# rsokolovskii/fl_scaling_sc_ldpc

Measured on AMD Instinct MI355X. Metric: MC codeword trials/sec, (4,8) SC-LDPC L=50 N=1000 eps=0.48 full BP, higher is better.
Workload: dtype u32

## Files before the change

### fl_scaling_sc_ldpc_amd/csrc/full_bp_small.hip

```cpp
#include "common.h"
#include "kernel_util.h"
#include "table_rows.h"
#include <algorithm>
#include <cstdlib>
#include <type_traits>

namespace {

using namespace scldpc_dev;

enum { SC_NE = 0, SC_REM, SC_N0, SC_N1, SC_OVF, SC_Q, SC_N = 8 };
enum { LV_VALID = 2, LV_EXTRA0 = 3, LV_PUSH = 6, LV_DROP = 9, LV_REM = 12, LV_OVF = 15, LV_N = 18 };

struct SmArgs {
    int L, V, C, n, nk, cn_lim, nw, ncw;
    uint32_t magic_v, magic_c;
    int ntrials;
    int kswitch;
    int max_it;
    int rows_cap;
    int32_t *rows;
    int off_U, off_q0, off_q1, off_pos, off_scal, off_fb, total, qcap;
    const uint16_t *vn_adj16;
    const uint16_t *cn_adj16;
    const uint32_t *chan;
    int32_t *counters;
    uint32_t *erased_out;
    int ncaps;
    int caps[SCLDPC_MAX_CAPS];
};


template <int BLOCK, bool LEVEL, bool PERSIST, bool SOCK, bool TRAJ = false, bool CAPS = false, bool WIDE = false, int DV = 4, int DC = 8,
          int OCC = 0>
__global__ __launch_bounds__(BLOCK, OCC ? OCC : WIDE ? 4 : PERSIST ? 8 : 7) __attribute__((amdgpu_num_sgpr(96))) void full_bp_small_kernel(const SmArgs a)
{
    static_assert(!WIDE || (BLOCK == 1024 && LEVEL && SOCK && !PERSIST), "the wide form: LEVEL [+ TRAJ | CAPS], socket table");
    static_assert(!(TRAJ && CAPS), "the checkpoints have no rows form");
    static_assert((DV == 4 && DC == 8) || (SOCK && !PERSIST), "other degree pairs: the socket table, no PERSIST");
    static_assert(DC <= 15 && DC % 2 == 0 && DV < DC, "a CN's count of erased neighbours is a nibble; CN rows are read as 32-bit words");
    using QT = std::conditional_t<WIDE, uint32_t, uint16_t>;
    constexpr int kWaves = BLOCK / 64;
    extern __shared__ uint32_t lds[];
    uint32_t *cnt = lds;
    uint32_t *U = lds + a.off_U;
    QT *q[2] = {reinterpret_cast<QT *>(lds + a.off_q0), reinterpret_cast<QT *>(lds + a.off_q1)};
    int *pos_cnt = reinterpret_cast<int *>(lds + a.off_pos);
    int *pos_ss = pos_cnt + a.L;
    int *scal = reinterpret_cast<int *>(lds + a.off_scal);

    const int tid = threadIdx.x, lane = tid & 63, wave = tid >> 6;
    auto decode_trial = [&](const int trial) {
    STAMP_DECL
    const int n = a.n, nk = a.nk, cn_lim = a.cn_lim, nw = a.nw, V = a.V, C = a.C, L = a.L, qcap = a.qcap;
    const auto *vrow = reinterpret_cast<const typename VnUnit<DV>::type *>(a.vn_adj16) + (size_t)trial * n * VnUnit<DV>::per_row;
    const auto *crow = reinterpret_cast<const typename CnUnit<DC>::type *>(a.cn_adj16) + (size_t)trial * nk * CnUnit<DC>::per_row;
    auto vn_row = [&](int j) { if constexpr (DV == 4) return load_row(vrow, j); else return load_row<DV>(vrow, j); };
    auto cn_row = [&](int c) { if constexpr (DC == 8) return load_row(crow, c); else return load_row<DC>(crow, c); };
    const uint32_t *ch = a.chan + (size_t)trial * nw;

    for (int c = tid; c < a.ncw; c += BLOCK) cnt[c] = 0;
    int ne_local = 0;
    for (int w = tid; w < nw; w += BLOCK) {
        const uint32_t x = chan_tail(ch[w], w, nw, n);
        U[w] = x;
        ne_local += __popc(x);
    }
    if (tid < LV_N) scal[tid] = 0;
    for (int i = tid; i < 2 * L; i += BLOCK) pos_cnt[i] = 0;
    __syncthreads();
    ne_local = wave_sum(ne_local);
    if (lane == 0 && ne_local) atomicAdd(&scal[SC_NE], ne_local);

    constexpr int NB = 8;
    for (int j0 = tid; j0 < n; j0 += NB * BLOCK) {
        Row<DV> r[NB];
        bool er[NB];
#pragma unroll
        for (int u = 0; u < NB; u++) {
            const int j = j0 + u * BLOCK;
            er[u] = false;
            if (j < n) { r[u] = vn_row(j); er[u] = (U[j >> 5] >> (j & 31)) & 1u; }
        }
#pragma unroll
        for (int u = 0; u < NB; u++) {
            const int j = j0 + u * BLOCK;
            if (er[u]) {
                const int base = (int)__umulhi((uint32_t)j, a.magic_v) * C;
                int cc[DV];
#pragma unroll
                for (int i = 0; i < DV; i++) cc[i] = base + i * C + (int)r[u][i];
#pragma unroll
                for (int i = 0; i < DV; i++) atomicAdd(&cnt[cc[i] >> 3], 1u << ((cc[i] & 7) * 4));
            }
        }
    }
    __syncthreads();
    STAMP(0);
    const int nch = scal[SC_NE];

    int removed = 0, drops = 0;
    auto step = [&](int c, uint32_t (&out)[DV]) {
#pragma unroll
        for (int i = 0; i < DV; i++) out[i] = 0;
        const Row<DC> s = cn_row(c);
        uint32_t jk[DC];
        bool none[DC];
#pragma unroll
        for (int k = 0; k < DC; k++) { jk[k] = s[k]; none[k] = jk[k] == 0xFFFFu; }
        if constexpr (SOCK) {
            const int vbase = (int)__umulhi((uint32_t)c, a.magic_c) * V;
#pragma unroll
            for (int k = 0; k < DC; k++) jk[k] = (uint32_t)(vbase - (int)(jk[k] % DV) * V) + (jk[k] / DV);
        }
        uint32_t wd[DC];
#pragma unroll
        for (int k = 0; k < DC; k++) wd[k] = U[none[k] ? 0u : jk[k] >> 5];
        int j = -1;
#pragma unroll
        for (int k = 0; k < DC; k++)
            if (!none[k] && ((wd[k] >> (jk[k] & 31u)) & 1u)) j = (int)jk[k];
        if (j < 0) return;
        const Row<DV> r = vn_row(j);
        const uint32_t bit = 1u << (j & 31);
        if (!(atomicAnd(&U[j >> 5], ~bit) & bit)) return;
        removed++;
        const int base = (int)__umulhi((uint32_t)j, a.magic_v) * C;
        int cc[DV];
#pragma unroll
        for (int i = 0; i < DV; i++) cc[i] = base + i * C + (int)r[i];
        uint32_t o[DV];
#pragma unroll
        for (int i = 0; i < DV; i++) o[i] = atomicSub(&cnt[cc[i] >> 3], 1u << ((cc[i] & 7) * 4));
#pragma unroll
        for (int i = 0; i < DV; i++) {
            const uint32_t old = (o[i] >> ((cc[i] & 7) * 4)) & 15u;
            if (old == 2u && cc[i] < cn_lim) out[i] = (uint32_t)cc[i] + 1u;
            if constexpr (LEVEL) drops += (old == 1u && cc[i] < cn_lim);
        }
    };
    auto ones_of = [&](int w) {
        const uint32_t y = cnt[w] ^ 0x11111111u;
        uint32_t z = ~(((y & 0x77777777u) + 0x77777777u) | y) & 0x88888888u;
        if (w * 8 + 8 > cn_lim) {
            const int keep = cn_lim - w * 8;
            z = keep <= 0 ? 0u : (z & ((1u << (4 * keep)) - 1u));
        }
        return z;
    };
    auto append = [&](const uint32_t (&out)[DV], int *push, QT *qn, bool &overflow) {
        int mine = 0;
#pragma unroll
        for (int i = 0; i < DV; i++) mine += out[i] != 0u;
        const int incl = (int)wave_inclusive_scan((uint32_t)mine);
        const int tot = __builtin_amdgcn_readlane(incl, 63);
        if (tot) {
            int base = 0;
            if (lane == 0) base = atomicAdd(push, tot);
            int idx = __builtin_amdgcn_readfirstlane(base) + incl - mine;
#pragma unroll
            for (int i = 0; i < DV; i++)
                if (out[i]) { if (idx < qcap) qn[idx] = (QT)(out[i] - 1u); else overflow = true; idx++; }
        }
    };

    int rounds = 0, ne = 0, status = 0, be = 0, ee = 0, bee = 0;
    auto residual = [&]() {
    if (ne > 0) {
        for (int w = tid; w < nw; w += BLOCK) {
            uint32_t x = U[w];
            int p0 = (int)__umulhi((uint32_t)(w * 32), a.magic_v);
            int room = (p0 + 1) * V - w * 32;
            while (x) {
                const uint32_t lo = room >= 32 ? x : (x & ((1u << room) - 1u));
                if (lo) atomicAdd(&pos_cnt[p0], __popc(lo));
                x = room >= 32 ? 0u : (x >> room);
                p0++;
                room = V;
            }
        }
        __syncthreads();
        int q0 = 0;
        for (;;) {
            while (q0 < L && pos_cnt[q0] == 0) q0++;
            if (q0 >= L) break;
            for (int t = tid; t < V; t += BLOCK) {
                const int j = q0 * V + t;
                if (!((U[j >> 5] >> (j & 31)) & 1u)) continue;
                const Row<DV> r = vn_row(j);
                const int base = q0 * C;
                int cc[DV];
#pragma unroll
                for (int i = 0; i < DV; i++) cc[i] = base + i * C + (int)r[i];
                bool pair = true;
#pragma unroll
                for (int i = 0; i < DV; i++) pair = pair && ((cnt[cc[i] >> 3] >> ((cc[i] & 7) * 4)) & 15u) == 2u;
                if (!pair) continue;
                int partner = -1;
                for (int i = 0; i < DV && pair; i++) {
                    const Row<DC> s = cn_row(cc[i]);
                    int other = -1;
                    for (int k = 0; k < DC; k++) {
                        const uint32_t jk = s[k];
                        if (jk == 0xFFFFu) continue;
                        const int j2 = SOCK ? (q0 + i - (int)(jk % DV)) * V + (int)(jk / DV) : (int)jk;
                        if (j2 != j && ((U[j2 >> 5] >> (j2 & 31)) & 1u)) other = j2;
                    }
                    if (other < 0 || (i > 0 && other != partner)) pair = false;
                    partner = other;
                }
                if (pair && (int)__umulhi((uint32_t)partner, a.magic_v) == q0) atomicAdd(&pos_ss[q0], 1);
            }
            __syncthreads();
            const int e = pos_cnt[q0] - pos_ss[q0];
            if (e > 0) { ee = e; bee = 1; break; }
            q0++;
        }
        for (int pos = 0; pos < L; pos++) be += pos_cnt[pos] > 0;
    }
    };
    auto put = [&](int32_t *o, int ne, int be, int ee, int bee, int rounds, int status) {
        o[SCLDPC_C_NUM_ERASURES] = ne;
        o[SCLDPC_C_NUM_BLOCKS_ERR] = be;
        o[SCLDPC_C_NUM_ERASURES_EXP] = ee;
        o[SCLDPC_C_NUM_BLOCKS_ERR_EXP] = bee;
        o[SCLDPC_C_NUM_ERASURES_P1] = 0;
        o[SCLDPC_C_ITERATIONS] = rounds;
        o[SCLDPC_C_STATUS] = status;
        o[SCLDPC_C_CHANNEL_ERASURES] = nch;
    };
    auto cap_counters = [&](int k) { return a.counters + ((size_t)k * a.ntrials + trial) * SCLDPC_NCOUNTERS; };

    int ci = 0;
    if constexpr (LEVEL) {
        uint8_t *fb = reinterpret_cast<uint8_t *>(lds + a.off_fb);
        int prec = n, iter = 0, ncur = 0, nfront = 0, first_word = 0;
        if constexpr (TRAJ) {
            int extra = 0;
            const int head = (DV - 1) * C, tail0 = L * C;
            for (int i = tid; i < 2 * head; i += BLOCK) {
                const int c = i < head ? i : tail0 + (i - head);
                if (c >= cn_lim || c >= nk) continue;
                const Row<DC> s = cn_row(c);
                int deg = 0;
#pragma unroll
                for (int k = 0; k < DC; k++) deg += s[k] != 0xFFFFu;
                extra += deg == 1 && ((cnt[c >> 3] >> ((c & 7) * 4)) & 15u) == 0u;
            }
            extra = wave_sum(extra);
            if (lane == 0 && extra) atomicAdd(&scal[LV_EXTRA0], extra);
        }
        bool scan = true;
        ne = nch;
        for (;;) {
            const int g = iter % 3, gn = (iter + 1) % 3;
            QT *qc = q[iter & 1], *qn = q[(iter + 1) & 1];
            if (tid == 0) { scal[LV_PUSH + gn] = 0; scal[LV_DROP + gn] = 0; scal[LV_REM + gn] = 0; scal[LV_OVF + gn] = 0; }
            int *push = &scal[LV_PUSH + g];
            bool overflow = false;
            removed = 0; drops = 0;
            auto run_queue = [&](int nq) {
                for (int k0 = wave * 64; k0 < nq; k0 += BLOCK) {
                    uint32_t out[DV] = {};
                    if (k0 + lane < nq) step((int)qc[k0 + lane], out);
                    append(out, push, qn, overflow);
                }
            };
            if (scan) {
                int valid = 0;
                for (int w = tid; w < a.ncw; w += BLOCK) {
                    uint32_t y = ones_of(w) >> 3;
                    y = (y | (y >> 3)) & 0x03030303u;
                    y = (y | (y >> 6)) & 0x000F000Fu;
                    y = (y | (y >> 12)) & 0xFFu;
                    fb[w] = (uint8_t)y;
                    valid += __popc(y);
                }
                if (iter == 0) {
                    valid = wave_sum(valid);
                    if (lane == 0 && valid) atomicAdd(&scal[LV_VALID], valid);
                }
                if (tid == 0) scal[SC_Q] = 0;
                __syncthreads();
                if (iter == 0) nfront = scal[LV_VALID];
                for (;;) {
                    for (int w0 = wave * 64; w0 < a.ncw; w0 += BLOCK) {
                        const int w = w0 + lane;
                        uint32_t y = w < a.ncw ? (uint32_t)fb[w] : 0u;
                        const int mine = __popc(y);
                        const int incl = (int)wave_inclusive_scan((uint32_t)mine);
                        const int tot = __builtin_amdgcn_readlane(incl, 63);
                        if (tot == 0) continue;
                        int base = 0;
                        if (lane == 0) base = atomicAdd(&scal[SC_Q], tot);
                        int idx = __builtin_amdgcn_readfirstlane(base) + incl - mine;
                        uint32_t left = 0;
                        while (y) {
                            const int k = __ffs((int)y) - 1;
                            y &= y - 1;
                            if (idx < qcap) qc[idx] = (QT)(w * 8 + k); else left |= 1u << k;
                            idx++;
                        }
                        if (mine) fb[w] = (uint8_t)left;
                    }
                    __syncthreads();
                    const int found = scal[SC_Q];
                    __syncthreads();
                    if (tid == 0) scal[SC_Q] = 0;
                    run_queue(min(found, qcap));
                    if (found <= qcap) break;
                    __syncthreads();
                }
            } else {
                run_queue(ncur);
            }
            STAMP(4);
            {
                const uint32_t both = (uint32_t)wave_sum((int)((uint32_t)removed | ((uint32_t)drops << 15)));
                removed = (int)(both & 0x7FFFu); drops = (int)(both >> 15);
            }
            if (lane == 0) {
                if (removed) atomicAdd(&scal[LV_REM + g], removed);
                if (drops) atomicAdd(&scal[LV_DROP + g], drops);
            }
            if (overflow) scal[LV_OVF + g] = 1;
            STAMP(5);
            __syncthreads();
            STAMP(6);
            const int deg1 = nfront + ((TRAJ && iter == 0) ? scal[LV_EXTRA0] : 0);
            ne -= scal[LV_REM + g];
            const int recovered = prec - ne;
            if constexpr (TRAJ) {
                if (wave == 0 && a.rows && rounds < a.rows_cap) {
                    int fw = first_word, first = n;
                    while (fw < nw) {
                        const uint32_t w = (fw + lane < nw) ? U[fw + lane] : 0u;
                        const unsigned long long m = __ballot(w != 0u);
                        if (m) {
                            const int l0 = __ffsll((long long)m) - 1;
                            const uint32_t w0 = (uint32_t)__shfl((int)w, l0, 64);
                            fw += l0;
                            first = fw * 32 + (__ffs((int)w0) - 1);
                            break;
                        }
                        fw += 64;
                    }
                    first_word = fw;
                    if (lane == 0) {
                        int32_t *r = a.rows + ((size_t)trial * a.rows_cap + rounds) * 3;
                        r[0] = deg1; r[1] = recovered; r[2] = (int)__umulhi((uint32_t)first, a.magic_v);
                    }
                }
                __syncthreads();
            }
            rounds++;
            if (deg1 < recovered && iter > 0) { status = -1; break; }
            if (ne == 0 || ne == prec) break;
            prec = ne;
            nfront = scal[LV_PUSH + g] - (scal[LV_DROP + g] - nfront);
            scan = scal[LV_OVF + g] != 0;
            ncur = scan ? 0 : scal[LV_PUSH + g];
            iter++;
            if (!CAPS && a.max_it > 0 && iter >= a.max_it) break;
            if constexpr (CAPS) {
                if (iter >= a.caps[ci]) {
                    be = ee = bee = 0;
                    residual();
                    if (tid == 0) put(cap_counters(ci), ne, be, ee, bee, rounds, 0);
                    __syncthreads();
                    for (int i = tid; i < 2 * L; i += BLOCK) pos_cnt[i] = 0;
                    if (++ci == a.ncaps) break;
                }
            }
            STAMP(7);
        }
        __syncthreads();
        STAMP(1);
    } else {
        const int kSwitch = a.kswitch;
        const int wcap = (qcap / kWaves) & ~1, half_cap = wcap / 2;
        int ncur = 0;
        bool scan = true;
        for (;;) {
            QT *qc = q[rounds & 1], *qn = q[(rounds + 1) & 1];
            if (scan) {
                for (int w0 = wave * 64; w0 < a.ncw; w0 += BLOCK) {
                    const int w = w0 + lane;
                    uint32_t z = w < a.ncw ? ones_of(w) : 0u;
                    const int mine = __popc(z);
                    const int incl = (int)wave_inclusive_scan((uint32_t)mine);
                    const int tot = __builtin_amdgcn_readlane(incl, 63);
                    if (tot == 0) continue;
                    int base = 0;
                    if (lane == 0) base = atomicAdd(&scal[SC_Q], tot);
                    base = __builtin_amdgcn_readfirstlane(base);
                    int idx = base + incl - mine;
                    while (z) {
                        const int k = (__ffs((int)z) - 1) >> 2;
                        z &= z - 1;
                        if (idx < qcap) qc[idx] = (QT)(w * 8 + k);
                        idx++;
                    }
                }
                __syncthreads();
                ncur = scal[SC_Q];
                if (ncur > qcap) { ncur = qcap; if (tid == 0) scal[SC_OVF] = 1; }
                __syncthreads();
            }
            if (tid == 0) { scal[SC_Q] = 0; scal[SC_N0 + ((rounds + 1) & 1)] = 0; }
            int *push = &scal[SC_N0 + (rounds & 1)];
            bool overflow = false;
            if (ncur > kSwitch || half_cap < 64) {
                for (int k0 = wave * 64; k0 < ncur; k0 += BLOCK) {
                    uint32_t out[DV] = {};
                    if (k0 + lane < ncur) step((int)qc[k0 + lane], out);
                    append(out, push, qn, overflow);
                }
            } else {
                QT *mine = qn + wave * wcap;
                int cntw = (ncur - wave + kWaves - 1) / kWaves, cur = 0;
                if (cntw < 0) cntw = 0;
                if (lane < cntw) mine[lane] = qc[wave + lane * kWaves];
                while (cntw > 0) {
                    QT *src = mine + cur * half_cap, *dst = mine + (cur ^ 1) * half_cap;
                    int ncnt = 0;
                    for (int b0 = 0; b0 < cntw; b0 += 64) {
                        uint32_t out[DV] = {};
                        if (b0 + lane < cntw) step((int)src[b0 + lane], out);
                        {
                            int mine_n = 0;
    #pragma unroll
                            for (int i = 0; i < DV; i++) mine_n += out[i] != 0u;
                            const int incl = (int)wave_inclusive_scan((uint32_t)mine_n);
                            int idx = ncnt + incl - mine_n;
    #pragma unroll
                            for (int i = 0; i < DV; i++)
                                if (out[i]) { if (idx < half_cap) dst[idx] = (QT)(out[i] - 1u); else overflow = true; idx++; }
                            ncnt += __builtin_amdgcn_readlane(incl, 63);
                        }
                    }
                    cntw = min(ncnt, half_cap);
                    cur ^= 1;
                }
            }
            if (overflow) scal[SC_OVF] = 1;
            __syncthreads();
            rounds++;
            const int pushed = *push;
            scan = scal[SC_OVF] != 0;
            __syncthreads();
            if (tid == 0) scal[SC_OVF] = 0;
            ncur = scan ? 0 : min(pushed, qcap);
            if (!scan && ncur == 0) break;
        }
        STAMP(1);
        removed = wave_sum(removed);
        if (lane == 0 && removed) atomicAdd(&scal[SC_REM], removed);
        __syncthreads();
        ne = nch - scal[SC_REM];
    }

    if (!CAPS || ci < a.ncaps) {
        be = ee = bee = 0;
        residual();
    }
    STAMP(2);
    STAMP_FLUSH();
    if (a.erased_out)
        for (int w = tid; w < nw; w += BLOCK) a.erased_out[(size_t)trial * nw + w] = U[w];
    if (tid == 0) {
        if constexpr (CAPS) {
            for (int k = ci; k < a.ncaps; k++) put(cap_counters(k), ne, be, ee, bee, rounds, status);
        } else {
            put(a.counters + (size_t)trial * SCLDPC_NCOUNTERS, ne, be, ee, bee, rounds, status);
        }
    }
    };
    if constexpr (PERSIST) {
        for (int trial = blockIdx.x; trial < a.ntrials; trial += gridDim.x) {
            decode_trial(trial);
            __syncthreads();
        }
    } else {
        decode_trial((int)blockIdx.x);
    }
}

int make_args(const scldpc_code_params *p, int32_t is_term, SmArgs *a, int per_cu, bool level = false, bool wide = false)
{
    const int n = scldpc::n_of(p), nk = scldpc::nk_of(p);
    a->L = p->L; a->V = p->vns_pos; a->C = p->cns_pos; a->n = n; a->nk = nk;
    a->cn_lim = is_term ? nk : p->L * p->cns_pos;
    a->nw = (n + 31) / 32; a->ncw = (nk + 7) / 8;
    int off = 0;
    auto take = [&](int words) { int o = off; off += (words + 3) & ~3; return o; };
    take(a->ncw);
    a->off_U = take(a->nw);
    a->off_pos = take(2 * p->L);
    a->off_scal = take(LV_N);
    a->off_fb = level ? take((a->ncw + 3) / 4) : 0;
    const int budget = scldpc::kMaxLdsBytes / per_cu / 4 - 128;
    int qwords = ((budget - off) / 2) & ~3;
    if (qwords > 2048 && !wide) qwords = 2048;
    if (qwords < 128) return -1;
    a->qcap = wide ? qwords : 2 * qwords;
    a->off_q0 = take(qwords);
    a->off_q1 = take(qwords);
    a->total = off;
    return 0;
}

constexpr int kBlockSmall = 256;
constexpr int kPerCu = 7;
constexpr int kSwitchWidth = 128;
constexpr int kBlockWide = 1024;
constexpr int kWideMinQueue = 1024;
static_assert(kSwitchWidth <= 64 * (kBlockSmall / 64), "a wave takes at most one frontier entry per lane into its private queue");

constexpr int pair_of(int dv, int dc) { return dv == 4 && dc == 8 ? 0 : dv == 3 && dc == 6 ? 1 : dv == 5 && dc == 10 ? 2 : -1; }

int carve(const scldpc_code_params *p, int32_t is_term, bool level, bool wide, SmArgs *a, int per_cu = kPerCu)
{
    if (wide) per_cu = 1;
    while (per_cu > 1 && make_args(p, is_term, a, per_cu, level, wide) != 0) per_cu--;
    return make_args(p, is_term, a, per_cu, level, wide) == 0 ? per_cu : -1;
}

const char *shape_limit(const scldpc_code_params *p, bool wide, bool sock, bool deg = false)
{
    if (scldpc::check_params(p)) return "invalid code parameters";
    if (!deg) {
        if (p->dv != 4 || p->dc != 8) return "takes dv = 4, dc = 8 only";
    } else {
        if (p->dc > 15) return "dc must be at most 15 (a CN's count of erased neighbours is kept in 4 bits)";
        if (pair_of(p->dv, p->dc) < 0) {
            static thread_local char text[96];
            snprintf(text, sizeof text, "no instance for dv = %d, dc = %d (takes (3,6), (4,8) and (5,10))", p->dv, p->dc);
            return text;
        }
    }
    if (sock && (int64_t)p->vns_pos * p->dv > 65535) return "sockets: vns_pos * dv must fit 16 bits (at most 65535)";
    if (p->cns_pos > 65536) return "at most 65536 CNs per position (16-bit position-local CN ids)";
    const int64_t n64 = (int64_t)p->L * p->vns_pos, nk64 = (int64_t)(p->L + p->dv - 1) * p->cns_pos;
    if (!wide && nk64 > 65536) return "at most 65536 CNs per trial (16-bit queue entries; the _wide forms take more)";
    if (!sock && n64 >= 65535) return "global VN ids in the CN -> VN table: fewer than 65535 VNs (use the _sock16 form beyond)";
    if (n64 / 8 + nk64 / 2 > scldpc::kMaxLdsBytes) return "LDS: the CN counts and VN bits of a trial exceed 160 KiB";
    SmArgs a{};
    uint32_t m;
    if (!scldpc::magic_of(p->vns_pos, scldpc::n_of(p) + 32, &m) || !scldpc::magic_of(p->cns_pos, scldpc::nk_of(p), &m))
        return "no exact multiply-high division for this vns_pos / cns_pos";
    if (make_args(p, 1, &a, 1, wide, wide) != 0) return "LDS: the CN counts and VN bits of a trial leave no room for the queues";
    if (wide && a.qcap < kWideMinQueue) return "queue: the LDS left by the state holds fewer than 1024 entries per queue";
    if (wide && a.nk / 16 + 64 * (a.nk / a.qcap + 1) > 32767) return "queue: a wave's releases per iteration could exceed 15 bits";
    if (deg) {
        if (!wide && carve(p, 1, true, false, &a) < 0) return "LDS: the CN counts and VN bits of a trial leave no room for the queues";
        const int r = a.nk / (wide ? kBlockWide / 64 : kBlockSmall / 64) + 64 * (a.nk / a.qcap + 1);
        if (r > 32767) return "queue: a wave's releases per iteration could exceed 15 bits";
        if (p->dv * r >= (1 << 17)) return "queue: the CNs a wave zeroes per iteration could exceed 17 bits";
    }
    return nullptr;
}

}

const char *scldpc::small_deg_shape_limit(const scldpc_code_params *p) { return shape_limit(p, false, true, true); }

extern "C" int scldpc_full_bp_wide_supported(const scldpc_code_params *p) { return shape_limit(p, true, true) == nullptr; }

extern "C" int scldpc_full_bp_cn16_supported(const scldpc_code_params *p) { return shape_limit(p, false, false) == nullptr; }

extern "C" int scldpc_full_bp_sock16_supported(const scldpc_code_params *p) { return shape_limit(p, false, true) == nullptr; }

namespace {

enum Mode { M_FIX, M_LEVEL, M_TRAJ, M_CAPS };
constexpr bool kCnTable = false, kSockTable = true, kNarrow = false, kWide = true, kDeg = true;
struct Form {
    Mode mode;
    bool sock;
    bool wide;
    bool deg = false;
    bool knobs() const { return mode != M_CAPS && !wide && !deg; }
};

struct Call {
    const scldpc_code_params *p;
    int32_t ntrials;
    const uint16_t *vn_adj16, *cn_adj16;
    const uint32_t *chan;
    int32_t max_it, is_term;
    int32_t *counters;
    uint32_t *erased;
    void *stream;
    int32_t *rows; int32_t rows_cap;
    int32_t ncaps; const int32_t *caps;
};

using Kernel = void (*)(const SmArgs);
constexpr int form_key(Mode mode, bool sock, bool wide, bool persist, int pair = 0)
{
    return pair * 32 + mode * 8 + sock * 4 + wide * 2 + persist;
}

Kernel kernel_of(const Form &f, bool persist, int pair = 0)
{
    constexpr int S = kBlockSmall, W = kBlockWide;
    switch (form_key(f.mode, f.sock, f.wide, persist, pair)) {
    case form_key(M_FIX, kCnTable, kNarrow, false):      return full_bp_small_kernel<S, false, false, false>;
    case form_key(M_FIX, kSockTable, kNarrow, false):    return full_bp_small_kernel<S, false, false, true>;
    case form_key(M_FIX, kCnTable, kNarrow, true):       return full_bp_small_kernel<S, false, true, false>;
    case form_key(M_LEVEL, kCnTable, kNarrow, false):    return full_bp_small_kernel<S, true, false, false>;
    case form_key(M_LEVEL, kSockTable, kNarrow, false):  return full_bp_small_kernel<S, true, false, true>;
    case form_key(M_LEVEL, kCnTable, kNarrow, true):     return full_bp_small_kernel<S, true, true, false>;
    case form_key(M_TRAJ, kCnTable, kNarrow, false):     return full_bp_small_kernel<S, true, false, false, true>;
    case form_key(M_TRAJ, kSockTable, kNarrow, false):   return full_bp_small_kernel<S, true, false, true, true>;
    case form_key(M_CAPS, kCnTable, kNarrow, false):     return full_bp_small_kernel<S, true, false, false, false, true>;
    case form_key(M_CAPS, kSockTable, kNarrow, false):   return full_bp_small_kernel<S, true, false, true, false, true>;
    case form_key(M_LEVEL, kSockTable, kWide, false):    return full_bp_small_kernel<W, true, false, true, false, false, true>;
    case form_key(M_TRAJ, kSockTable, kWide, false):     return full_bp_small_kernel<W, true, false, true, true, false, true>;
    case form_key(M_FIX, kSockTable, kNarrow, false, 1):   return full_bp_small_kernel<S, false, false, true, false, false, false, 3, 6>;
    case form_key(M_LEVEL, kSockTable, kNarrow, false, 1): return full_bp_small_kernel<S, true, false, true, false, false, false, 3, 6>;
    case form_key(M_TRAJ, kSockTable, kNarrow, false, 1):  return full_bp_small_kernel<S, true, false, true, true, false, false, 3, 6>;
    case form_key(M_LEVEL, kSockTable, kWide, false, 1):   return full_bp_small_kernel<W, true, false, true, false, false, true, 3, 6>;
    case form_key(M_TRAJ, kSockTable, kWide, false, 1):    return full_bp_small_kernel<W, true, false, true, true, false, true, 3, 6>;
    case form_key(M_FIX, kSockTable, kNarrow, false, 2):   return full_bp_small_kernel<S, false, false, true, false, false, false, 5, 10>;
    case form_key(M_LEVEL, kSockTable, kNarrow, false, 2): return full_bp_small_kernel<S, true, false, true, false, false, false, 5, 10>;
    case form_key(M_TRAJ, kSockTable, kNarrow, false, 2):  return full_bp_small_kernel<S, true, false, true, true, false, false, 5, 10, 6>;
    case form_key(M_LEVEL, kSockTable, kWide, false, 2):   return full_bp_small_kernel<W, true, false, true, false, false, true, 5, 10>;
    case form_key(M_TRAJ, kSockTable, kWide, false, 2):    return full_bp_small_kernel<W, true, false, true, true, false, true, 5, 10>;
    case form_key(M_CAPS, kSockTable, kWide, false):       return full_bp_small_kernel<W, true, false, true, false, true, true>;
    case form_key(M_CAPS, kSockTable, kNarrow, false, 1):  return full_bp_small_kernel<S, true, false, true, false, true, false, 3, 6>;
    case form_key(M_CAPS, kSockTable, kNarrow, false, 2):  return full_bp_small_kernel<S, true, false, true, false, true, false, 5, 10>;
    case form_key(M_CAPS, kSockTable, kWide, false, 1):    return full_bp_small_kernel<W, true, false, true, false, true, true, 3, 6>;
    case form_key(M_CAPS, kSockTable, kWide, false, 2):    return full_bp_small_kernel<W, true, false, true, false, true, true, 5, 10>;
    }
    return nullptr;
}

int per_cu_of(const Form &f, int pair) { return f.wide ? 1 : (pair == pair_of(5, 10) && f.mode == M_TRAJ) ? 6 : kPerCu; }

int launch(const char *who, const Form &f, const Call &c)
{
    if (int rc = scldpc::check_params(c.p)) return rc;
    if (c.rows && c.rows_cap <= 0) return scldpc::set_error(SCLDPC_ERR_BAD_ARG, "%s: d_rows given but rows_cap <= 0", who);
    if (f.mode == M_CAPS) {
        if (c.ncaps < 1 || c.ncaps > SCLDPC_MAX_CAPS || !c.caps)
            return scldpc::set_error(SCLDPC_ERR_BAD_ARG, "%s: takes 1 .. %d caps (ncaps = %d%s)", who, SCLDPC_MAX_CAPS, c.ncaps,
                                     c.caps ? "" : ", caps NULL");
        for (int k = 0; k < c.ncaps; k++)
            if (c.caps[k] < 1 || (k > 0 && c.caps[k] <= c.caps[k - 1]))
                return scldpc::set_error(SCLDPC_ERR_BAD_ARG, "%s: caps must be strictly increasing and >= 1 (caps[%d] = %d)", who,
                                         k, c.caps[k]);
    }
    if (const char *why = shape_limit(c.p, f.wide, f.sock, f.deg)) return scldpc::set_error(SCLDPC_ERR_TOO_LARGE, "%s: %s", who, why);
    if (c.ntrials < 0 || (c.ntrials > 0 && (!c.counters || !c.vn_adj16 || !c.cn_adj16 || !c.chan)))
        return scldpc::set_error(SCLDPC_ERR_BAD_ARG, "%s: null buffer or negative ntrials", who);
    if (c.ntrials == 0) return SCLDPC_OK;

    SmArgs a{};
    const int pair = f.deg ? pair_of(c.p->dv, c.p->dc) : 0;
    if (carve(c.p, c.is_term, f.mode != M_FIX, f.wide, &a, per_cu_of(f, pair)) < 0)
        return scldpc::set_error(SCLDPC_ERR_TOO_LARGE, "%s: LDS: the CN counts and VN bits do not fit", who);
    scldpc::magic_of(c.p->vns_pos, a.n + 32, &a.magic_v);
    scldpc::magic_of(c.p->cns_pos, a.nk, &a.magic_c);
    a.vn_adj16 = c.vn_adj16; a.cn_adj16 = c.cn_adj16; a.chan = c.chan;
    a.counters = c.counters; a.erased_out = c.erased;
    a.ntrials = c.ntrials;
    a.max_it = c.max_it;
    a.rows = c.rows; a.rows_cap = c.rows ? c.rows_cap : 0;
    a.ncaps = c.ncaps;
    for (int k = 0; k < c.ncaps; k++) a.caps[k] = c.caps[k];
    a.kswitch = kSwitchWidth;
    int grid = c.ntrials;
    size_t lds_bytes = 4u * (size_t)a.total;
    if (f.knobs()) {
        if (const char *v = getenv("SCLDPC_DEBUG_DECODER_KSWITCH")) a.kswitch = std::min(atoi(v), 64 * (kBlockSmall / 64));
        grid = scldpc::debug_grid("DECODER", c.ntrials);
        lds_bytes = std::min(lds_bytes + scldpc::debug_lds_pad("DECODER"), (size_t)scldpc::kMaxLdsBytes);
    }
    if (f.sock && grid < c.ntrials)
        return scldpc::set_error(SCLDPC_ERR_BAD_ARG, "%s: no persistent form with the socket table", who);
    const Kernel kern = kernel_of(f, grid < c.ntrials && f.mode != M_TRAJ, pair);
    if (int rc = scldpc::allow_max_lds(reinterpret_cast<const void *>(kern))) return rc;
    hipLaunchKernelGGL(kern, dim3(grid), dim3(f.wide ? kBlockWide : kBlockSmall), lds_bytes, static_cast<hipStream_t>(c.stream), a);
    SCLDPC_HIP_CHECK(hipGetLastError());
    return SCLDPC_OK;
}

}

extern "C" int scldpc_full_bp_fixpoint_device_cn16(const scldpc_code_params *p, int32_t ntrials,
                                                   const uint16_t *d_vn_adj16, const uint16_t *d_cn_adj16,
                                                   const uint32_t *d_chan_bits, int32_t is_term, int32_t *d_counters,
                                                   uint32_t *d_erased_bits, void *stream)
{
    return launch("scldpc_full_bp_fixpoint_device_cn16", {M_FIX, kCnTable, kNarrow},
                  {p, ntrials, d_vn_adj16, d_cn_adj16, d_chan_bits, 0, is_term, d_counters, d_erased_bits, stream});
}

extern "C" int scldpc_full_bp_device_cn16(const scldpc_code_params *p, int32_t ntrials, const uint16_t *d_vn_adj16,
                                          const uint16_t *d_cn_adj16, const uint32_t *d_chan_bits, int32_t max_it,
                                          int32_t is_term, int32_t *d_counters, uint32_t *d_erased_bits, void *stream)
{
    return launch("scldpc_full_bp_device_cn16", {M_LEVEL, kCnTable, kNarrow},
                  {p, ntrials, d_vn_adj16, d_cn_adj16, d_chan_bits, max_it, is_term, d_counters, d_erased_bits, stream});
}

extern "C" int scldpc_full_bp_fixpoint_device_sock16(const scldpc_code_params *p, int32_t ntrials,
                                                     const uint16_t *d_vn_adj16, const uint16_t *d_cn_sock16,
                                                     const uint32_t *d_chan_bits, int32_t is_term, int32_t *d_counters,
                                                     uint32_t *d_erased_bits, void *stream)
{
    return launch("scldpc_full_bp_fixpoint_device_sock16", {M_FIX, kSockTable, kNarrow},
                  {p, ntrials, d_vn_adj16, d_cn_sock16, d_chan_bits, 0, is_term, d_counters, d_erased_bits, stream});
}

extern "C" int scldpc_full_bp_device_sock16(const scldpc_code_params *p, int32_t ntrials, const uint16_t *d_vn_adj16,
                                            const uint16_t *d_cn_sock16, const uint32_t *d_chan_bits, int32_t max_it,
                                            int32_t is_term, int32_t *d_counters, uint32_t *d_erased_bits, void *stream)
{
    return launch("scldpc_full_bp_device_sock16", {M_LEVEL, kSockTable, kNarrow},
                  {p, ntrials, d_vn_adj16, d_cn_sock16, d_chan_bits, max_it, is_term, d_counters, d_erased_bits, stream});
}

extern "C" int scldpc_full_bp_traj_device_cn16(const scldpc_code_params *p, int32_t ntrials, const uint16_t *d_vn_adj16,
                                               const uint16_t *d_cn_adj16, const uint32_t *d_chan_bits, int32_t max_it,
                                               int32_t is_term, int32_t *d_counters, int32_t *d_rows, int32_t rows_cap,
                                               uint32_t *d_erased_bits, void *stream)
{
    if (!d_rows) return scldpc::set_error(SCLDPC_ERR_BAD_ARG, "scldpc_full_bp_traj_device_cn16: null d_rows");
    return launch("scldpc_full_bp_traj_device_cn16", {M_TRAJ, kCnTable, kNarrow},
                  {p, ntrials, d_vn_adj16, d_cn_adj16, d_chan_bits, max_it, is_term, d_counters, d_erased_bits, stream, d_rows, rows_cap});
}

extern "C" int scldpc_full_bp_traj_device_sock16(const scldpc_code_params *p, int32_t ntrials, const uint16_t *d_vn_adj16,
                                                 const uint16_t *d_cn_sock16, const uint32_t *d_chan_bits, int32_t max_it,
                                                 int32_t is_term, int32_t *d_counters, int32_t *d_rows, int32_t rows_cap,
                                                 uint32_t *d_erased_bits, void *stream)
{
    if (!d_rows) return scldpc::set_error(SCLDPC_ERR_BAD_ARG, "scldpc_full_bp_traj_device_sock16: null d_rows");
    return launch("scldpc_full_bp_traj_device_sock16", {M_TRAJ, kSockTable, kNarrow},
                  {p, ntrials, d_vn_adj16, d_cn_sock16, d_chan_bits, max_it, is_term, d_counters, d_erased_bits, stream, d_rows, rows_cap});
}

extern "C" int scldpc_full_bp_caps_device_cn16(const scldpc_code_params *p, int32_t ntrials, const uint16_t *d_vn_adj16,
                                               const uint16_t *d_cn_adj16, const uint32_t *d_chan_bits, int32_t ncaps,
                                               const int32_t *caps, int32_t is_term, int32_t *d_counters, void *stream)
{
    return launch("scldpc_full_bp_caps_device_cn16", {M_CAPS, kCnTable, kNarrow},
                  {p, ntrials, d_vn_adj16, d_cn_adj16, d_chan_bits, 0, is_term, d_counters, nullptr, stream, nullptr, 0, ncaps, caps});
}

extern "C" int scldpc_full_bp_caps_device_sock16(const scldpc_code_params *p, int32_t ntrials, const uint16_t *d_vn_adj16,
                                                 const uint16_t *d_cn_sock16, const uint32_t *d_chan_bits, int32_t ncaps,
                                                 const int32_t *caps, int32_t is_term, int32_t *d_counters, void *stream)
{
    return launch("scldpc_full_bp_caps_device_sock16", {M_CAPS, kSockTable, kNarrow},
                  {p, ntrials, d_vn_adj16, d_cn_sock16, d_chan_bits, 0, is_term, d_counters, nullptr, stream, nullptr, 0, ncaps, caps});
}

extern "C" int scldpc_full_bp_device_wide(const scldpc_code_params *p, int32_t ntrials, const uint16_t *d_vn_adj16,
                                          const uint16_t *d_cn_sock16, const uint32_t *d_chan_bits, int32_t max_it,
                                          int32_t is_term, int32_t *d_counters, uint32_t *d_erased_bits, void *stream)
{
    return launch("scldpc_full_bp_device_wide", {M_LEVEL, kSockTable, kWide},
                  {p, ntrials, d_vn_adj16, d_cn_sock16, d_chan_bits, max_it, is_term, d_counters, d_erased_bits, stream});
}

extern "C" int scldpc_full_bp_traj_device_wide(const scldpc_code_params *p, int32_t ntrials, const uint16_t *d_vn_adj16,
                                               const uint16_t *d_cn_sock16, const uint32_t *d_chan_bits, int32_t max_it,
                                               int32_t is_term, int32_t *d_counters, int32_t *d_rows, int32_t rows_cap,
                                               uint32_t *d_erased_bits, void *stream)
{
    if (!d_rows) return scldpc::set_error(SCLDPC_ERR_BAD_ARG, "scldpc_full_bp_traj_device_wide: null d_rows");
    return launch("scldpc_full_bp_traj_device_wide", {M_TRAJ, kSockTable, kWide},
                  {p, ntrials, d_vn_adj16, d_cn_sock16, d_chan_bits, max_it, is_term, d_counters, d_erased_bits, stream, d_rows, rows_cap});
}

extern "C" int scldpc_full_bp_caps_device_wide(const scldpc_code_params *p, int32_t ntrials, const uint16_t *d_vn_adj16,
                                               const uint16_t *d_cn_sock16, const uint32_t *d_chan_bits, int32_t ncaps,
                                               const int32_t *caps, int32_t is_term, int32_t *d_counters, void *stream)
{
    return launch("scldpc_full_bp_caps_device_wide", {M_CAPS, kSockTable, kWide},
                  {p, ntrials, d_vn_adj16, d_cn_sock16, d_chan_bits, 0, is_term, d_counters, nullptr, stream, nullptr, 0, ncaps, caps});
}

extern "C" int scldpc_full_bp_deg_supported(const scldpc_code_params *p) { return shape_limit(p, false, true, true) == nullptr; }

extern "C" int scldpc_full_bp_deg_wide_supported(const scldpc_code_params *p) { return shape_limit(p, true, true, true) == nullptr; }

extern "C" int scldpc_full_bp_fixpoint_device_deg(const scldpc_code_params *p, int32_t ntrials, const uint16_t *d_vn_adj16,
                                                  const uint16_t *d_cn_sock16, const uint32_t *d_chan_bits, int32_t is_term,
                                                  int32_t *d_counters, uint32_t *d_erased_bits, void *stream)
{
    return launch("scldpc_full_bp_fixpoint_device_deg", {M_FIX, kSockTable, kNarrow, kDeg},
                  {p, ntrials, d_vn_adj16, d_cn_sock16, d_chan_bits, 0, is_term, d_counters, d_erased_bits, stream});
}

extern "C" int scldpc_full_bp_device_deg(const scldpc_code_params *p, int32_t ntrials, const uint16_t *d_vn_adj16,
                                         const uint16_t *d_cn_sock16, const uint32_t *d_chan_bits, int32_t max_it,
                                         int32_t is_term, int32_t *d_counters, uint32_t *d_erased_bits, void *stream)
{
    return launch("scldpc_full_bp_device_deg", {M_LEVEL, kSockTable, kNarrow, kDeg},
                  {p, ntrials, d_vn_adj16, d_cn_sock16, d_chan_bits, max_it, is_term, d_counters, d_erased_bits, stream});
}

extern "C" int scldpc_full_bp_traj_device_deg(const scldpc_code_params *p, int32_t ntrials, const uint16_t *d_vn_adj16,
                                              const uint16_t *d_cn_sock16, const uint32_t *d_chan_bits, int32_t max_it,
                                              int32_t is_term, int32_t *d_counters, int32_t *d_rows, int32_t rows_cap,
                                              uint32_t *d_erased_bits, void *stream)
{
    if (!d_rows) return scldpc::set_error(SCLDPC_ERR_BAD_ARG, "scldpc_full_bp_traj_device_deg: null d_rows");
    return launch("scldpc_full_bp_traj_device_deg", {M_TRAJ, kSockTable, kNarrow, kDeg},
                  {p, ntrials, d_vn_adj16, d_cn_sock16, d_chan_bits, max_it, is_term, d_counters, d_erased_bits, stream, d_rows, rows_cap});
}

extern "C" int scldpc_full_bp_device_deg_wide(const scldpc_code_params *p, int32_t ntrials, const uint16_t *d_vn_adj16,
                                              const uint16_t *d_cn_sock16, const uint32_t *d_chan_bits, int32_t max_it,
                                              int32_t is_term, int32_t *d_counters, uint32_t *d_erased_bits, void *stream)
{
    return launch("scldpc_full_bp_device_deg_wide", {M_LEVEL, kSockTable, kWide, kDeg},
                  {p, ntrials, d_vn_adj16, d_cn_sock16, d_chan_bits, max_it, is_term, d_counters, d_erased_bits, stream});
}

extern "C" int scldpc_full_bp_traj_device_deg_wide(const scldpc_code_params *p, int32_t ntrials, const uint16_t *d_vn_adj16,
                                                   const uint16_t *d_cn_sock16, const uint32_t *d_chan_bits, int32_t max_it,
                                                   int32_t is_term, int32_t *d_counters, int32_t *d_rows, int32_t rows_cap,
                                                   uint32_t *d_erased_bits, void *stream)
{
    if (!d_rows) return scldpc::set_error(SCLDPC_ERR_BAD_ARG, "scldpc_full_bp_traj_device_deg_wide: null d_rows");
    return launch("scldpc_full_bp_traj_device_deg_wide", {M_TRAJ, kSockTable, kWide, kDeg},
                  {p, ntrials, d_vn_adj16, d_cn_sock16, d_chan_bits, max_it, is_term, d_counters, d_erased_bits, stream, d_rows, rows_cap});
}

extern "C" int scldpc_full_bp_caps_device_deg(const scldpc_code_params *p, int32_t ntrials, const uint16_t *d_vn_adj16,
                                              const uint16_t *d_cn_sock16, const uint32_t *d_chan_bits, int32_t ncaps,
                                              const int32_t *caps, int32_t is_term, int32_t *d_counters, void *stream)
{
    return launch("scldpc_full_bp_caps_device_deg", {M_CAPS, kSockTable, kNarrow, kDeg},
                  {p, ntrials, d_vn_adj16, d_cn_sock16, d_chan_bits, 0, is_term, d_counters, nullptr, stream, nullptr, 0, ncaps, caps});
}

extern "C" int scldpc_full_bp_caps_device_deg_wide(const scldpc_code_params *p, int32_t ntrials, const uint16_t *d_vn_adj16,
                                                   const uint16_t *d_cn_sock16, const uint32_t *d_chan_bits, int32_t ncaps,
                                                   const int32_t *caps, int32_t is_term, int32_t *d_counters, void *stream)
{
    return launch("scldpc_full_bp_caps_device_deg_wide", {M_CAPS, kSockTable, kWide, kDeg},
                  {p, ntrials, d_vn_adj16, d_cn_sock16, d_chan_bits, 0, is_term, d_counters, nullptr, stream, nullptr, 0, ncaps, caps});
}
```

Baseline: 1.248 million.

## Replace per-wave level-synchronous tail with persistent per-lane work-stealing stack

In the narrow-frontier tail phase, each wave now keeps one check node per lane and follows one newly released node locally. Extra released nodes go onto a per-wave LDS stack, and idle lanes refill from it through a ballot and mbcnt rank. Row loads are prefetched for the next node. This replaces the double-buffered per-wave queue rounds and is meant to cut the idle lanes and round overhead of small frontiers, at the cost of divergent control flow and more wave barriers. A debug env knob to cap qcap is also added.

New measurement: 1.259 million, median of 6. About the same (+0.8%).

```diff
diff --git a/fl_scaling_sc_ldpc_amd/csrc/full_bp_small.hip b/fl_scaling_sc_ldpc_amd/csrc/full_bp_small.hip
--- a/fl_scaling_sc_ldpc_amd/csrc/full_bp_small.hip
+++ b/fl_scaling_sc_ldpc_amd/csrc/full_bp_small.hip
@@ -100,10 +100,9 @@
     const int nch = scal[SC_NE];
 
     int removed = 0, drops = 0;
-    auto step = [&](int c, uint32_t (&out)[DV]) {
+    auto release = [&](int c, const Row<DC> &s, uint32_t (&out)[DV]) {
 #pragma unroll
         for (int i = 0; i < DV; i++) out[i] = 0;
-        const Row<DC> s = cn_row(c);
         uint32_t jk[DC];
         bool none[DC];
 #pragma unroll
@@ -139,6 +138,7 @@
             if constexpr (LEVEL) drops += (old == 1u && cc[i] < cn_lim);
         }
     };
+    auto step = [&](int c, uint32_t (&out)[DV]) { release(c, cn_row(c), out); };
     auto ones_of = [&](int w) {
         const uint32_t y = cnt[w] ^ 0x11111111u;
         uint32_t z = ~(((y & 0x77777777u) + 0x77777777u) | y) & 0x88888888u;
@@ -378,7 +378,7 @@
         STAMP(1);
     } else {
         const int kSwitch = a.kswitch;
-        const int wcap = (qcap / kWaves) & ~1, half_cap = wcap / 2;
+        const int wcap = qcap / kWaves;
         int ncur = 0;
         bool scan = true;
         for (;;) {
@@ -410,37 +410,50 @@
             if (tid == 0) { scal[SC_Q] = 0; scal[SC_N0 + ((rounds + 1) & 1)] = 0; }
             int *push = &scal[SC_N0 + (rounds & 1)];
             bool overflow = false;
-            if (ncur > kSwitch || half_cap < 64) {
+            if (ncur > kSwitch) {
                 for (int k0 = wave * 64; k0 < ncur; k0 += BLOCK) {
                     uint32_t out[DV] = {};
                     if (k0 + lane < ncur) step((int)qc[k0 + lane], out);
                     append(out, push, qn, overflow);
                 }
             } else {
-                QT *mine = qn + wave * wcap;
-                int cntw = (ncur - wave + kWaves - 1) / kWaves, cur = 0;
-                if (cntw < 0) cntw = 0;
-                if (lane < cntw) mine[lane] = qc[wave + lane * kWaves];
-                while (cntw > 0) {
-                    QT *src = mine + cur * half_cap, *dst = mine + (cur ^ 1) * half_cap;
-                    int ncnt = 0;
-                    for (int b0 = 0; b0 < cntw; b0 += 64) {
-                        uint32_t out[DV] = {};
-                        if (b0 + lane < cntw) step((int)src[b0 + lane], out);
-                        {
-                            int mine_n = 0;
-    #pragma unroll
-                            for (int i = 0; i < DV; i++) mine_n += out[i] != 0u;
-                            const int incl = (int)wave_inclusive_scan((uint32_t)mine_n);
-                            int idx = ncnt + incl - mine_n;
-    #pragma unroll
-                            for (int i = 0; i < DV; i++)
-                                if (out[i]) { if (idx < half_cap) dst[idx] = (QT)(out[i] - 1u); else overflow = true; idx++; }
-                            ncnt += __builtin_amdgcn_readlane(incl, 63);
-                        }
+                QT *stk = reinterpret_cast<QT *>(lds + (((rounds + 1) & 1) ? a.off_q1 : a.off_q0)) + wave * wcap;
+                uint32_t mycn = 0;
+                int sp = 0;
+                bool popped = false;
+                Row<DC> s = {}, s2 = {};
+                if (wave + lane * kWaves < ncur) { mycn = (uint32_t)qc[wave + lane * kWaves] + 1u; s = cn_row((int)mycn - 1); }
+                while (__ballot(mycn != 0u)) {
+                    uint32_t out[DV] = {};
+                    if (popped) s = s2;
+                    if (mycn) release((int)mycn - 1, s, out);
+                    mycn = 0;
+                    int extras = 0;
+#pragma unroll
+                    for (int i = 0; i < DV; i++) {
+                        const bool first = out[i] != 0u && mycn == 0u;
+                        mycn = first ? out[i] : mycn;
+                        out[i] = first ? 0u : out[i];
+                        extras += out[i] != 0u;
                     }
-                    cntw = min(ncnt, half_cap);
-                    cur ^= 1;
+                    if (mycn) s = cn_row((int)mycn - 1);
+                    popped = false;
+                    if (__ballot(extras > 0)) {
+                        const int incl = (int)wave_inclusive_scan((uint32_t)extras);
+                        int idx = sp + incl - extras;
+#pragma unroll
+                        for (int i = 0; i < DV; i++)
+                            if (out[i]) { if (idx < wcap) stk[idx] = (QT)(out[i] - 1u); else overflow = true; idx++; }
+                        sp = min(sp + __builtin_amdgcn_readlane(incl, 63), wcap);
+                    }
+                    if (sp > 0) {
+                        __builtin_amdgcn_wave_barrier();
+                        const unsigned long long idle = __ballot(mycn == 0u);
+                        const int k = (int)__builtin_amdgcn_mbcnt_hi((uint32_t)(idle >> 32), __builtin_amdgcn_mbcnt_lo((uint32_t)idle, 0u));
+                        if (mycn == 0u && k < sp) { mycn = (uint32_t)stk[sp - 1 - k] + 1u; s2 = cn_row((int)mycn - 1); popped = true; }
+                        sp -= min(sp, (int)__popcll(idle));
+                        __builtin_amdgcn_wave_barrier();
+                    }
                 }
             }
             if (overflow) scal[SC_OVF] = 1;
@@ -515,7 +528,7 @@
 constexpr int kSwitchWidth = 128;
 constexpr int kBlockWide = 1024;
 constexpr int kWideMinQueue = 1024;
-static_assert(kSwitchWidth <= 64 * (kBlockSmall / 64), "a wave takes at most one frontier entry per lane into its private queue");
+static_assert(kSwitchWidth <= 64 * (kBlockSmall / 64), "a wave takes at most one frontier entry per lane in its private phase");
 
 constexpr int pair_of(int dv, int dc) { return dv == 4 && dc == 8 ? 0 : dv == 3 && dc == 6 ? 1 : dv == 5 && dc == 10 ? 2 : -1; }
 
@@ -675,6 +688,7 @@
     size_t lds_bytes = 4u * (size_t)a.total;
     if (f.knobs()) {
         if (const char *v = getenv("SCLDPC_DEBUG_DECODER_KSWITCH")) a.kswitch = std::min(atoi(v), 64 * (kBlockSmall / 64));
+        if (const char *v = getenv("SCLDPC_DEBUG_DECODER_QCAP")) a.qcap = std::min(a.qcap, 2 * std::clamp(atoi(v), 128, 1 << 20));
         grid = scldpc::debug_grid("DECODER", c.ntrials);
         lds_bytes = std::min(lds_bytes + scldpc::debug_lds_pad("DECODER"), (size_t)scldpc::kMaxLdsBytes);
     }
```
